# dfm/tinygp

Hardware: AMD Instinct MI355X
Metric: GP log_probability evals/sec + Cholesky TFLOP/s (fp64), N=16,384 (higher is better)
Workload: dtype f64; 1 GPU; c2: 1.5^2 ExpSquared(2.5), 1-D X, N=16384, fp64, diag=0.01, constant-density synthetic inputs (SURVEY 8d), dense Cholesky + tri-solve; n=16384, d=1, parallelism=single, nb_outer=1024

## Files before the change

### tinygp_amd/csrc/capi.hip

```cpp
#include <cmath>
#include <cstdlib>
#include <chrono>
#include <cstring>
#include <string>

#include "tgp_common.h"
#define CHAIN_HD __host__ __device__
#include "chain_tasks.h"
#define TILE_HD
#include "tile_order.h"

namespace tgp {

static thread_local std::string g_error;

void set_error(const char* fmt, ...) {
  char buf[1024];
  va_list ap;
  va_start(ap, fmt);
  vsnprintf(buf, sizeof(buf), fmt, ap);
  va_end(ap);
  g_error = buf;
}

// ... 35 lines not shown
struct tgp_solver {
  tgp_ctx* ctx = nullptr;
  int dtype = TGP_F64;
  int64_t n = 0, npad = 0;
  int d = 1;
  void* X = nullptr;
  void* diag = nullptr;
  void* A = nullptr;
  void* dinv = nullptr;
  void* vec = nullptr;
  void* vec2 = nullptr;
  void* resid = nullptr;
  void* scratch = nullptr;
  void* Minv = nullptr;
  void* winv = nullptr;
  bool winv_valid = false;
  size_t scratch_bytes = 0;
  KProg kp{};
  bool has_prog = false, factored = false, has_resid = false;
  int32_t info = 0;
  double logdet_half = 0;
  double ms[8] = {0, 0, 0, 0, 0, 0, 0, 0};
};

#define CTX_GUARD(ctx)                                                \
  TGP_ARG_CHECK((ctx) != nullptr, "null context");                    \
  std::unique_lock<std::recursive_mutex> _tgp_lock((ctx)->mu);        \
  TGP_HIP_TRY(hipSetDevice((ctx)->device))

#define SOLVER_GUARD(s)                                               \
  TGP_ARG_CHECK((s) != nullptr && (s)->ctx != nullptr, "null solver"); \
  std::unique_lock<std::recursive_mutex> _tgp_lock((s)->ctx->mu);     \
  TGP_HIP_TRY(hipSetDevice((s)->ctx->device))

template <typename T>
static int assemble_lower(tgp_ctx* ctx, const tgp::KProg& kp, int64_t n, int d, const T* X,
                          const T* diag, T* A, int64_t npad) {
  using namespace tgp;
  const int64_t tc = npad / 128;
  int64_t t1 = tc;
  if (ctx->lookahead != 0 && ctx->asm_stream != nullptr) {
    int64_t nb = ctx->nb_outer / 128;
    if (nb < 1) nb = 1;
    nb = std::max<int64_t>(nb, first_panel_cols(ctx, npad) / 128);
    if (nb < tc) t1 = nb;
  }
  const int flags = KMAT_LOWER | KMAT_PAD_IDENTITY;
  if (t1 < tc) {
    TGP_TRY(ev_record(ctx, ctx->ev_asm, ctx->stream));
    TGP_TRY(st_wait(ctx, ctx->asm_stream, ctx->ev_asm));
  }
  TGP_TRY(launch_kmat_cols<T>(ctx, ctx->stream, kp, n, n, d, X, X, diag, A, npad, npad, npad, flags, 0, t1));
  if (t1 < tc) {
    auto side = [=]() -> int {
      TGP_TRY(launch_kmat_cols<T>(ctx, ctx->asm_stream, kp, n, n, d, X, X, diag, A, npad, npad, npad,
                                  flags, t1, tc - t1));
      return ev_record(ctx, ctx->ev_asm, ctx->asm_stream);
    };
    if (ctx->asm_defer != 0) {
      ctx->deferred_asm = side;
    } else {
      TGP_TRY(side());
    }
    ctx->asm_pending = true;
  }
  return TGP_OK;
}

template <typename T>
static int ensure_winv(tgp_solver* s) {
  if (s->winv_valid) return TGP_OK;
// ... 167 lines not shown
  if (!strcmp(key, "chain_batch_minrows")) return &ctx->chain_batch_minrows;
  if (!strcmp(key, "kmat_plain_div")) return &ctx->kmat_plain_div;
  if (!strcmp(key, "chain_reserve")) return &ctx->chain_reserve;
  if (!strcmp(key, "gate_split")) return &ctx->gate_split;
  if (!strcmp(key, "reserve_max_tiles")) return &ctx->reserve_max_tiles;
  if (!strcmp(key, "sub_panel")) return &ctx->sub_panel;
  if (!strcmp(key, "sub_panel_min_rows")) return &ctx->sub_panel_min_rows;
  if (!strcmp(key, "nb_first")) return &ctx->nb_first;
  if (!strcmp(key, "split_tail")) return &ctx->split_tail;
  if (!strcmp(key, "gemm_role")) return &ctx->gemm_role;
  if (!strcmp(key, "host_join")) return &ctx->host_join;
  if (!strcmp(key, "late_join")) return &ctx->late_join;
  if (!strcmp(key, "chain_reduce")) return &ctx->chain_reduce;
  if (!strcmp(key, "asm_defer")) return &ctx->asm_defer;
  if (!strcmp(key, "tile_band")) return &ctx->tile_band;
  if (!strcmp(key, "fault_inject")) return &ctx->fault_inject;
  if (!strcmp(key, "poll_timeout_ms")) return &ctx->poll_timeout_ms;
  if (!strcmp(key, "timeout_retries")) return &ctx->timeout_retries;
  return nullptr;
}

static int set_option_checked(tgp_ctx* ctx, const char* key, int64_t value, int64_t* old) {
  int64_t* slot = option_slot(ctx, key);
  TGP_ARG_CHECK(slot != nullptr, "unknown option '%s'", key);
  if (slot == &ctx->nb_outer)
    TGP_ARG_CHECK(value >= TILE && value % TILE == 0, "nb_outer must be a positive multiple of %d", TILE);
  if (slot == &ctx->sub_panel || slot == &ctx->nb_first)
    TGP_ARG_CHECK(value >= 0 && value % TILE == 0, "%s must be a multiple of %d (0: off)", key, TILE);
  if (slot == &ctx->chain_batch) TGP_ARG_CHECK(value >= 0 && value <= 32, "chain_batch must be in [0, 32]");
  if (slot == &ctx->chain_batch_lag) TGP_ARG_CHECK(value >= 1 && value <= 64, "chain_batch_lag must be in [1, 64]");
// ... 245 lines not shown
  s->n = n;
  s->npad = round_up(n, TILE);
  s->d = d;
  const size_t es = esize(dtype);
  auto fail = [&](int code) { tgp_solver_destroy(s); return code; };
#define S_TRY(expr) do { hipError_t _e = (expr); if (_e != hipSuccess) { \
    set_error("%s failed: %s", #expr, hipGetErrorString(_e));            \
    return fail(_e == hipErrorOutOfMemory ? TGP_E_NOMEM : TGP_E_HIP); } } while (0)
  S_TRY(hipMalloc(&s->X, size_t(n) * d * es));
  S_TRY(hipMalloc(&s->diag, size_t(n) * es));
  S_TRY(hipMalloc(&s->A, size_t(s->npad) * s->npad * es));
  S_TRY(hipMalloc(&s->dinv, size_t(s->npad / TILE) * 2048 * es));
  S_TRY(hipMalloc(&s->vec, size_t(s->npad) * es));
  S_TRY(hipMalloc(&s->vec2, size_t(s->npad) * es));
  S_TRY(hipMalloc(&s->resid, size_t(s->npad) * es));
  S_TRY(hipMemcpyAsync(s->X, X_host, size_t(n) * d * es, hipMemcpyHostToDevice, ctx->stream));
  S_TRY(hipMemcpyAsync(s->diag, noise_diag_host, size_t(n) * es, hipMemcpyHostToDevice, ctx->stream));
  S_TRY(hipMemsetAsync(s->vec, 0, size_t(s->npad) * es, ctx->stream));
  S_TRY(hipMemsetAsync(s->vec2, 0, size_t(s->npad) * es, ctx->stream));
  S_TRY(hipMemsetAsync(s->resid, 0, size_t(s->npad) * es, ctx->stream));
  S_TRY(hipStreamSynchronize(ctx->stream));
#undef S_TRY
  *out = s;
  return TGP_OK;
}

int tgp_solver_destroy(tgp_solver* s) {
  if (!s) return TGP_OK;
  if (s->ctx) {
    hipSetDevice(s->ctx->device);
    hipStreamSynchronize(s->ctx->stream);
  }
  void* bufs[] = {s->X, s->diag, s->A, s->dinv, s->vec, s->vec2, s->resid, s->scratch, s->Minv, s->winv};
  for (void* b : bufs)
    if (b) hipFree(b);
  delete s;
  return TGP_OK;
}

int tgp_solver_set_noise(tgp_solver* s, const void* noise_diag_host) {
  SOLVER_GUARD(s);
  TGP_ARG_CHECK(noise_diag_host != nullptr, "null input array");
  TGP_HIP_TRY(hipMemcpyAsync(s->diag, noise_diag_host, size_t(s->n) * esize(s->dtype),
                             hipMemcpyHostToDevice, s->ctx->stream));
  TGP_HIP_TRY(hipStreamSynchronize(s->ctx->stream));
  return TGP_OK;
}

// ... 61 lines not shown
    TGP_HIP_TRY(hipEventCreate(&e2));
    TGP_HIP_TRY(hipEventRecord(e0, ctx->stream));
  }
  int status = dispatch(s->dtype, [&](auto tag) {
    using T = decltype(tag);
    T* A = (T*)s->A;
    if (fused) {
      if (resid_host) {
        TGP_TRY(upload_vec(s, s->vec, resid_host));
      } else {
        TGP_ARG_CHECK(s->has_resid, "no resident residual: call tgp_solver_set_resid first");
        TGP_HIP_TRY(hipMemcpyAsync(s->vec, s->resid, size_t(s->npad) * es, hipMemcpyDeviceToDevice,
                                   ctx->stream));
      }
    }
    if (cov_host != nullptr) {
      TGP_TRY(solver_scratch(s, size_t(s->n) * s->n * es));
      TGP_HIP_TRY(hipMemcpyAsync(s->scratch, cov_host, size_t(s->n) * s->n * es,
                                 hipMemcpyHostToDevice, ctx->stream));
      TGP_TRY(launch_set_lower_from_rowmajor<T>(ctx, s->n, s->npad, (const T*)s->scratch, A, s->npad));
    } else {
      TGP_TRY(assemble_lower<T>(ctx, s->kp, s->n, s->d, (const T*)s->X, (const T*)s->diag, A, s->npad));
    }
    if (prof) TGP_HIP_TRY(hipEventRecord(e1, ctx->stream));
    int32_t inf = 0;
    ctx->defer_join = ctx->late_join != 0;
    ctx->join_deferred = false;
    reductions_begin(ctx, s->npad, fused != 0);
    int st = potrf<T>(ctx, s->npad, A, s->npad, (T*)s->dinv, &inf, fused ? (T*)s->vec : (T*)nullptr);
    ctx->defer_join = false;
    const bool reduce = reductions_end(ctx);
    if (st < 0) return st;
    s->info = inf;
    if (prof) TGP_HIP_TRY(hipEventRecord(e2, ctx->stream));
    if (reduce) {
      TGP_TRY(launch_sum_log_diag<T>(ctx, s->n, A, s->npad, 1));
      if (fused) TGP_TRY(launch_sum_squares<T>(ctx, s->n, (const T*)s->vec, 0));
    }
    return TGP_OK;
  });
  if (status < 0) return status;
  double two[2] = {0, 0};
  int32_t inf_late = 0;
  const bool late = ctx->join_deferred;
// ... 582 lines not shown
```

### tinygp_amd/csrc/chol.hip

```cpp
#include <algorithm>
#include <atomic>
#include <functional>
#include <type_traits>

#include <thread>

#include "tgp_common.h"
#define CHAIN_HD __host__ __device__
#include "chain_tasks.h"

namespace tgp {

namespace {

typedef double d4 __attribute__((ext_vector_type(4)));
typedef float f4 __attribute__((ext_vector_type(4)));

template <typename T> struct Mfma;
template <> struct Mfma<double> {
  using acc_t = d4;
  static __device__ __forceinline__ acc_t mma(double a, double b, acc_t c) {
    return __builtin_amdgcn_mfma_f64_16x16x4f64(a, b, c, 0, 0, 0);
  }
  static __device__ __forceinline__ int drow(int lane, int r) { return (lane >> 4) + 4 * r; }
// ... 2318 lines not shown
      TGP_TRY(launch_trsv_fwd_step<T>(ctx, S2, mb, Ljj, ld, dj, y + j0));
    }
    if (need_mid) TGP_TRY(mid(ctx->ev_d));
    if (SB > 0 && j0 + TILE == sub_end && sub_end < k0 + kb) {
      const int64_t s0 = sub_end - SB, mr = n - sub_end, ncr = k0 + kb - sub_end;
      const T* P = A + s0 * ld + sub_end;
      const int64_t tiles = (mr / TILE) * (ncr / TILE) - (ncr / TILE) * (ncr / TILE - 1) / 2;
      TGP_TRY(launch_gemm_nt<T>(ctx, st, mr, ncr, SB, P, ld, P, ld, A + sub_end * ld + sub_end, ld, 1, 0,
                                tiles <= ctx->first_small_tiles ? 4 : 1));
    }
  }
  return TGP_OK;
}

template <typename T>
int potrf(tgp_ctx* ctx, int64_t n, T* A, int64_t ld, T* dinv, int32_t* info_host, T* y) {
  TGP_ARG_CHECK(n % TILE == 0 && ld >= n, "potrf: n must be a multiple of %d and ld >= n", TILE);
  if (info_host) *info_host = 0;
  if (n == 0) return TGP_OK;
  ctx->potf2_wait_counter = nullptr;
  ctx->prefix_hint_cols = 0;
  ctx->prefix_hint_counter = nullptr;
  ctx->reserve_hint = 0;
  hipStream_t S0 = ctx->stream, S1 = ctx->panel_stream;
  if (ctx->solve_on_update == 0 && y != nullptr) TGP_TRY(ensure_solve_stream(ctx));
  hipStream_t S2 = ctx->solve_on_update != 0 ? ctx->update_stream : ctx->solve_stream;
  if (y != nullptr) {
    TGP_TRY(ev_record(ctx, ctx->ev_c, S0));
    TGP_TRY(st_wait(ctx, S2, ctx->ev_c));
  }
  int64_t NB = ctx->nb_outer;
  if (NB < TILE) NB = TILE;
  NB = NB / TILE * TILE;
  if (!ctx->trace) TGP_HIP_TRY(hipMemsetAsync(ctx->d_info, 0, sizeof(int32_t), S0));
  ctx->chain_stamp_base = 0;
  ctx->chain_launches = 0;
  ctx->chain_polls_pending = false;
  const bool prof_on = ctx->profile != 0 && !ctx->trace;
// ... 9 lines not shown
  auto potf2_at = [&](hipStream_t st, int64_t j0, bool pend) -> int {
    return panel_potf2<T>(ctx, st, A, ld, dinv, 0, j0, pend);
  };
  auto panel = [&](hipStream_t st, int64_t k0, int64_t kb, bool head_done, int64_t after_blocks,
                   const std::function<int(hipEvent_t)>& mid) -> int {
    return panel_chain<T>(ctx, st, n, A, ld, dinv, 0, k0, kb, head_done, y, after_blocks, mid);
  };
  const std::function<int(hipEvent_t)> no_mid = [](hipEvent_t) { return TGP_OK; };
  auto trailing = [&](hipStream_t sq, int64_t m, int64_t nn, int64_t kb, const T* P, T* C, int role) -> int {
    ProfSpan sp{};
    const bool prof = prof_on && role != 4 && role != 5;
    if (prof) {
      TGP_TRY(prof_event(ctx, &sp.e0));
      TGP_TRY(prof_event(ctx, &sp.e1));
      TGP_HIP_TRY(hipEventRecord(sp.e0, sq));
    }
    TGP_TRY(launch_gemm_nt<T>(ctx, sq, m, nn, kb, P, ld, P, ld, C, ld, 1, 0, role));
    if (prof) {
      TGP_HIP_TRY(hipEventRecord(sp.e1, sq));
      const double entries = double(nn) * double(m) - double(nn) * double(nn - 1) / 2.0;
      sp.flops = 2.0 * entries * double(kb);
      spans.push_back(sp);
    }
    return TGP_OK;
  };

  auto join_assembly = [&]() -> int {
    TGP_TRY(run_deferred_asm(ctx, nullptr));
    if (ctx->asm_pending) {
      TGP_TRY(st_wait(ctx, S0, ctx->ev_asm));
// ... 524 lines not shown
}

#define TGP_INST(T)                                                                              \
  template int spd_inverse_lower<T>(tgp_ctx*, int64_t, const T*, int64_t, const T*, T*, int64_t); \
  template int symmetrize_lower<T>(tgp_ctx*, int64_t, T*, int64_t);                               \
  template int launch_potf2<T>(tgp_ctx*, hipStream_t, T*, int64_t, T*, int32_t*, int32_t,       \
                               const T*, int64_t);       \
  template int launch_trsm<T>(tgp_ctx*, hipStream_t, int64_t, const T*, int64_t, const T*, T*,   \
                              int64_t);                                                          \
  template int launch_panel_step<T>(tgp_ctx*, hipStream_t, int64_t, T*, int64_t, T*, int32_t*, int32_t, \
                                    const T*, bool);                                             \
  template int compute_dinv<T>(tgp_ctx*, int64_t, const T*, int64_t, T*);                        \
  template int panel_potf2<T>(tgp_ctx*, hipStream_t, T*, int64_t, T*, int64_t, int64_t, bool);   \
  template int panel_chain<T>(tgp_ctx*, hipStream_t, int64_t, T*, int64_t, T*, int64_t, int64_t, \
                              int64_t, bool, T*, int64_t, const std::function<int(hipEvent_t)>&, int64_t, int64_t); \
  template int potrf<T>(tgp_ctx*, int64_t, T*, int64_t, T*, int32_t*, T*);                           \
  template int trsv<T>(tgp_ctx*, int64_t, const T*, int64_t, const T*, int, T*, const T*, const T*); \
  template int compute_winv<T>(tgp_ctx*, int64_t, const T*, int64_t, T*);                        \
  template int gemv_sub<T>(tgp_ctx*, int64_t, int64_t, const T*, int64_t, const T*, T*);                          \
  template int trsm_right_lt<T>(tgp_ctx*, int64_t, int64_t, const T*, int64_t, const T*, T*,     \
                                int64_t);
TGP_INST(float)
TGP_INST(double)
#undef TGP_INST

}
```

### tinygp_amd/csrc/gemm.hip

```cpp
#include <type_traits>

#include "tgp_common.h"

#define TILE_HD __host__ __device__
#include "tile_order.h"

namespace tgp {

namespace {

typedef double d4 __attribute__((ext_vector_type(4)));
typedef float f4 __attribute__((ext_vector_type(4)));

template <typename T> struct Mfma;
template <> struct Mfma<double> {
  using acc_t = d4;
  using v2_t = double __attribute__((ext_vector_type(2)));
  static __device__ __forceinline__ acc_t mma(double a, double b, acc_t c) {
    return __builtin_amdgcn_mfma_f64_16x16x4f64(a, b, c, 0, 0, 0);
  }
  static __device__ __forceinline__ int drow(int lane, int r) { return (lane >> 4) + 4 * r; }
};
template <> struct Mfma<float> {
  using acc_t = f4;
// ... 15 lines not shown
  int tm, tn;
  int k;
  int lower;
  int mode;
  int nblk;
  int skip00;
  int dG, dr, dl0, dnbt;
  int split_first, split_s, ngrid;
  T* ws;
  int* cnt;
  int batch;
  int64_t sA, sB, sC;
  int band;
  int prefix_tn = 0, prefix_cnt = 0;
  int32_t* prefix_done = nullptr;
};

__device__ __forceinline__ void decode_tile(int b, int tm, int tn, int lower, int& ti, int& tj, int band = 0) {
  tile_decode(b, tm, tn, lower, band, ti, tj);
}

template <typename T>
__device__ __forceinline__ void decode_tile_dist(int b, const GemmArgs<T>& g, int& ti, int& tj, int& gt) {
  int q = 0, g0 = (g.dl0 * g.dG + g.dr) * g.dnbt;
  const int step = g.dG * g.dnbt, tri = g.dnbt * (g.dnbt - 1) / 2;
  for (;;) {
    const int cnt = g.dnbt * (g.tm - g0) - tri;
    if (b < cnt) break;
    b -= cnt;
    g0 += step;
    ++q;
// ... 72 lines not shown
      ti += g.prefix_tn;
      tj += g.prefix_tn;
    }
    gt = tj;
  } else {
    decode_tile(bid, g.tm, g.tn, g.lower, ti, tj, g.band);
    gt = tj;
  }

  const int tid = threadIdx.x, lane = tid & 63, w = tid >> 6;
  const int wr = w >> 1, wc = w & 1;
  const int64_t i0 = int64_t(ti) * BM, j0 = int64_t(tj) * BN;

  int nkt = (g.mode & 2) ? ((g.k < (tj + 1) * BN ? g.k : (tj + 1) * BN) / BK) : g.k / BK;
  if (ROLE == 3 && (g.mode & 8)) nkt = (g.k < (ti + 1) * BM ? g.k : (ti + 1) * BM) / BK;
  const int kt0 = (g.mode & 4) ? (ti * BM) / BK : 0;
  const bool krev = ROLE == 3 && (g.mode & 16);
  const int lrow = lane & 15, lk = lane >> 4;
  T* Cb = gC + (j0 + wc * 64) * g.ldc + i0 + wr * 64;

  if constexpr (sizeof(T) == 8) {
    const int lq = (lane >> 2) & 3, lj = lane & 3;
    double acc[4][4][4];
#pragma unroll
    for (int a = 0; a < 4; ++a)
#pragma unroll
      for (int b = 0; b < 4; ++b)
#pragma unroll
        for (int t = 0; t < 4; ++t) acc[a][b][t] = 0.0;
    int rot[4];
#pragma unroll
    for (int t = 0; t < 4; ++t) rot[t] = 4 * ((lq + t) & 3) + lj;

    constexpr int NCH = 8;
    const int kq = (nkt - kt0) / nsl;
    const int kbeg = kt0 + slice * kq, kend = kbeg + kq;
    const bool pipe = (g.mode == 0) && nsl == 1 && (kend - kbeg >= NCH);
    double cst[8];
    const int wu = __builtin_amdgcn_readfirstlane(w);
    const char* Cu = reinterpret_cast<const char*>(gC + (j0 + (wu & 1) * 64) * g.ldc + i0 + (wu >> 1) * 64);
    uint32_t voff[4];
#pragma unroll
    for (int t = 0; t < 4; ++t) voff[t] = uint32_t((int64_t(4 * lq + lk) * g.ldc + rot[t]) * 8);
    const uint32_t lds_a = uint32_t(size_t((__attribute__((address_space(3))) T*)(&sA[0][0]))) + uint32_t(wu * LDS_LD * 8);
    const uint32_t lds_b = uint32_t(size_t((__attribute__((address_space(3))) T*)(&sB[0][0]))) + uint32_t(wu * LDS_LD * 8);
    const T* Au = gA + i0;
    const T* Bu = gB + int64_t(gt) * BN;
    const uint32_t lane16 = uint32_t(lane) * 16u;
    auto issue_tile = [&](int kt_, int buf_) {
      const int64_t kg = int64_t(krev ? kbeg + kend - 1 - kt_ : kt_) * BK + wu;
#pragma unroll
// ... 38 lines not shown
#pragma unroll
            for (int t = 0; t < 4; ++t)
              acc[a][b][t] = __builtin_amdgcn_mfma_f64_4x4x4f64(aop[a], bop[t], acc[a][b][t], 0, 0, NEG);
        }
      }
      tile_landed();
      __syncthreads();
      if constexpr (c >= 0) {
        __builtin_amdgcn_sched_barrier(0);
#pragma unroll
        for (int bb = 0; bb < 2; ++bb)
#pragma unroll
          for (int t = 0; t < 4; ++t) acc[c >> 1][(c & 1) * 2 + bb][t] += cst[bb * 4 + t];
      }
    };
    issue_tile(kbeg, kbeg & 1);
    tile_landed();
    __syncthreads();
    int kt = kbeg;
    if (pipe) {
      int one = 1;
      asm volatile("" : "+s"(one));
#define TGP_STAGED(C) \
  for (int q = 0; q < one; ++q, ++kt) ktile(kt, std::integral_constant<int, C>{}, std::true_type{});
      TGP_STAGED(0) TGP_STAGED(1) TGP_STAGED(2) TGP_STAGED(3) TGP_STAGED(4)
      TGP_STAGED(5) TGP_STAGED(6) TGP_STAGED(7)
#undef TGP_STAGED
      for (; kt < kend; ++kt) ktile(kt, std::integral_constant<int, -1>{}, std::true_type{});
    } else {
      for (; kt < kend; ++kt) ktile(kt, std::integral_constant<int, -1>{}, std::false_type{});
    }
// ... 481 lines not shown
static unsigned persistent_grid(const tgp_ctx* ctx, int nblk, int64_t reserve) {
  if (reserve <= 0) return unsigned(nblk);
  int64_t slots = 2 * int64_t(ctx->cus > 0 ? ctx->cus : 256) - reserve;
  slots = slots / 8 * 8;
  if (slots < 8) slots = 8;
  return unsigned(nblk <= slots ? nblk : slots);
}

template <typename T>
int launch_gemm_nt(tgp_ctx* ctx, hipStream_t st, int64_t m, int64_t n, int64_t k, const T* A,
                   int64_t lda, const T* B, int64_t ldb, T* C, int64_t ldc, int lower, int mode,
                   int role) {
  TGP_ARG_CHECK(m % BM == 0 && n % BN == 0 && k % BK == 0 && k > 0,
                "gemm_nt: m,n must be multiples of %d and k of %d (got %lld,%lld,%lld)", BM, BK,
                (long long)m, (long long)n, (long long)k);
  if (m == 0 || n == 0) return TGP_OK;
  if (ctx->trace) {
    const int64_t pfx = role == 0 ? ctx->prefix_hint_cols / BN : 0;
    ctx->prefix_hint_cols = 0;
    ctx->prefix_hint_counter = nullptr;
    if (role == 0) ctx->reserve_hint = 0;
    trace_push(ctx, 3, st, trace_off(ctx, A), trace_off(ctx, B), trace_off(ctx, C), m, n, k,
               int64_t(lower) | (int64_t(role) << 8) | (pfx << 16), ldc);
    return TGP_OK;
  }
  GemmArgs<T> g;
  g.skip00 = 0;
  g.dG = g.dr = g.dl0 = g.dnbt = 0;
  g.split_first = 0; g.split_s = 1; g.ngrid = 0; g.ws = nullptr; g.cnt = nullptr;
  g.batch = 1; g.sA = g.sB = g.sC = 0;
// ... 27 lines not shown
  } else {
    g.nblk = g.tm * g.tn;
  }
  const int64_t reserve = role == 0 ? ctx->reserve_hint : 0;
  ctx->reserve_hint = 0;
  if (role == 0 && ctx->prefix_hint_cols > 0) {
    TGP_ARG_CHECK(lower && mode == 0 && m == n && ctx->prefix_hint_cols % BN == 0 && ctx->prefix_hint_cols < n &&
                      k / BK >= 8 && ctx->prefix_hint_counter != nullptr,
                  "gemm_nt: a prefix needs a lower square update with at least 128 k-columns");
    g.prefix_tn = int(ctx->prefix_hint_cols / BN);
    g.prefix_cnt = tile_count(g.tm, g.prefix_tn, 1);
    g.prefix_done = ctx->prefix_hint_counter;
  }
  ctx->prefix_hint_cols = 0;
  ctx->prefix_hint_counter = nullptr;
  g.split_first = g.nblk; g.split_s = 1; g.ngrid = g.nblk; g.ws = nullptr; g.cnt = nullptr;
  if (ctx->split_tail != 0 && role == 0 && mode == 0 && reserve <= 0 && sizeof(T) == 8 && st == ctx->stream && g.prefix_cnt == 0) {
    const int slots = 2 * (ctx->cus > 0 ? ctx->cus : 256);
    const int R = g.nblk % slots, nkt = g.k / BK;
    int S = 1;
    while (R > 0 && 2 * S * R <= slots && 2 * S <= 8 && nkt % (2 * S) == 0 && nkt / (2 * S) >= 8) S *= 2;
    if (S > 1) {
      const size_t need = size_t(slots) * BM * BN * sizeof(T) + size_t(slots) * sizeof(int);
      if (ctx->gemm_ws_bytes < need) {
        if (ctx->d_gemm_ws) TGP_HIP_TRY(hipFree(ctx->d_gemm_ws));
        ctx->d_gemm_ws = nullptr;
        ctx->gemm_ws_bytes = 0;
        TGP_HIP_TRY(hipMalloc(&ctx->d_gemm_ws, need));
        TGP_HIP_TRY(hipMemset(ctx->d_gemm_ws, 0, need));
        ctx->gemm_ws_bytes = need;
// ... 136 lines not shown
```

### tinygp_amd/csrc/kmat.hip

```cpp
#include <algorithm>

#include "tgp_common.h"

namespace tgp {

namespace {

template <typename T> struct MathC;
template <> struct MathC<double> {
  static constexpr double SQRT3 = 1.7320508075688772;
  static constexpr double SQRT5 = 2.23606797749979;
  static constexpr double PI = 3.141592653589793;
  static constexpr double TWO_PI = 6.283185307179586;
};
template <> struct MathC<float> {
  static constexpr float SQRT3 = 1.7320508075688772f;
  static constexpr float SQRT5 = 2.23606797749979f;
  static constexpr float PI = 3.141592653589793f;
  static constexpr float TWO_PI = 6.283185307179586f;
};

template <typename T, int FAM = 0>
__device__ __forceinline__ T leaf_value(const KProg& kp, int i, T r1, T r2, T r3 = T(0)) {
  const int op = kp.op[i];
// ... 278 lines not shown
      const T a = MathC<T>::SQRT3 * by_p0.template div<FAST>(dist);
      return (T(1) + a) * exp(-a);
    } else {
      const T a = MathC<T>::SQRT5 * by_p0.template div<FAST>(dist);
      return (T(1) + a + by3.template div<FAST>(a * a)) * exp(-a);
    }
  }
}

template <typename T, int OP, int L2>
__device__ __forceinline__ T leaf_fast(T r1, T r2, T p0, T p0sq) {
  const UDiv<T> by_p0(p0), by_p0sq(p0sq), by3(T(3));
  return leaf_fast<T, OP, L2, false>(r1, r2, by_p0, by_p0sq, by3);
}

template <typename T, int D, int OP, int L2>
__global__ __launch_bounds__(256) void kmat_fast_kernel(T p0, T amp, int64_t n1, int64_t n2,
                                                        const T* __restrict__ X1,
                                                        const T* __restrict__ X2,
                                                        const T* __restrict__ diag, T* __restrict__ out,
                                                        int64_t ld, int flags, int tc0, int tri_h) {
  typedef T T2 __attribute__((ext_vector_type(2)));
  constexpr int NCOL = 32;
  const int cq = threadIdx.x >> 6, l = threadIdx.x & 63;
  int tr, tc;
  if (flags & KMAT_LOWER) {
    const int b = blockIdx.x;
    const double h2 = 2.0 * tri_h + 1.0;
    int j = int((h2 - sqrt(h2 * h2 - 8.0 * double(b))) * 0.5);
    while (j > 0 && j * tri_h - j * (j - 1) / 2 > b) --j;
    while ((j + 1) * tri_h - (j + 1) * j / 2 <= b) ++j;
    tc = tc0 + j;
    tr = tc + (b - (j * tri_h - j * (j - 1) / 2));
  } else {
    tr = blockIdx.x;
    tc = blockIdx.y + tc0;
// ... 2 lines not shown
  for (int t = threadIdx.x; t < KT * D; t += 256) s2all[t] = X2[int64_t(tc) * KT * D + t];
  __syncthreads();
  const T* s2 = s2all + cq * NCOL * D;
  const int64_t c0 = int64_t(tc) * KT + cq * NCOL;
  const int64_t gi = int64_t(tr) * KT + 2 * l;
  T xr[2][D];
#pragma unroll
  for (int h = 0; h < 2; ++h)
#pragma unroll
    for (int t = 0; t < D; ++t) xr[h][t] = X1[(gi + h) * D + t];
  const bool on_diag = diag != nullptr && tr == tc;
  const T dg0 = on_diag ? diag[gi] : T(0), dg1 = on_diag ? diag[gi + 1] : T(0);
  const UDiv<T> by_p0(p0), by_p0sq(p0 * p0), by3(T(3));
  const int ldiag = 2 * l - cq * NCOL;
  T* o = out + c0 * ld + gi;
  auto columns = [&](auto fast) -> T {
    constexpr bool FAST = decltype(fast)::value;
    T seen = 0;
#pragma unroll 4
    for (int c = 0; c < NCOL; ++c) {
      T v[2];
#pragma unroll
      for (int h = 0; h < 2; ++h) {
        T r1 = 0, r2 = 0;
#pragma unroll
        for (int t = 0; t < D; ++t) {
          const T dx = xr[h][t] - s2[c * D + t];
          r1 += fabs(dx);
          r2 += dx * dx;
        }
        v[h] = amp * leaf_fast<T, OP, L2, FAST>(r1, r2, by_p0, by_p0sq, by3);
        if constexpr (FAST) seen = fmax(seen, L2 ? r2 : r1);
      }
      if (on_diag) {
        if (c == ldiag) v[0] += dg0;
        if (c == ldiag + 1) v[1] += dg1;
      }
      T2 pair;
      pair.x = v[0];
      pair.y = v[1];
      *reinterpret_cast<T2*>(o + int64_t(c) * ld) = pair;
    }
    return seen;
  };
  bool plain = true;
  if (sizeof(T) == 8 && !(flags & KMAT_PLAIN_DIV) && by_p0.exact && by_p0sq.exact) {
    plain = !(columns(std::true_type{}) <= T(0x1p300));
  }
  if (plain) columns(std::false_type{});
}

template <typename T, int D, int FAM>
__global__ __launch_bounds__(256) void kmat_kernel(KProg kp, int64_t n1, int64_t n2, int d,
                                                   const T* __restrict__ X1,
                                                   const T* __restrict__ X2,
                                                   const T* __restrict__ diag, T* __restrict__ out,
                                                   int64_t ld, int64_t rows_out, int64_t cols_out,
                                                   int flags, int tc0, int ftr, int ftc) {
  const int tr = blockIdx.x, tc = blockIdx.y + tc0;
  if ((flags & KMAT_LOWER) && tr < tc) return;
  if (tr < ftr && tc < ftc) return;
  extern __shared__ __attribute__((aligned(16))) char smem[];
  T* s1 = reinterpret_cast<T*>(smem);
  T* s2 = s1 + KT * d;
  const int64_t r0 = int64_t(tr) * KT, c0 = int64_t(tc) * KT;
  load_tile_pair(s1, s2, X1, X2, r0, c0, n1, n2, d);

  const int il = threadIdx.x & (KT - 1);
  const int g = threadIdx.x >> 7;
  const int64_t gi = r0 + il;
  T xr[D > 0 ? D : 1];
  if constexpr (D > 0) {
#pragma unroll
    for (int t = 0; t < D; ++t) xr[t] = s1[il * D + t];
  }
  const T dg = (diag != nullptr && gi < n1) ? diag[gi] : T(0);
  if (gi >= rows_out) return;
  for (int c = 0; c < KT / 2; ++c) {
    const int jl = g * (KT / 2) + c;
    const int64_t gj = c0 + jl;
    if (gj >= cols_out) break;
    T v;
    if (gi < n1 && gj < n2) {
      T r1, r2, r3;
      if constexpr (D > 0) pair_dist<T, FAM, D>(xr, s2 + jl * D, d, r1, r2, r3);
      else pair_dist<T, FAM, 0>(s1 + il * d, s2 + jl * d, d, r1, r2, r3);
      v = eval_kprog<T, FAM>(kp, r1, r2, r3);
      if (diag != nullptr && gi == gj) v += dg;
    } else {
      v = ((flags & KMAT_PAD_IDENTITY) && gi == gj) ? T(1) : T(0);
    }
    out[gj * ld + gi] = v;
  }
}

template <typename T, int OP, int L2>
__device__ __forceinline__ T leaf_deriv_fast(T r1, T r2, T p0) {
  if constexpr (OP == TGP_K_EXPSQ) {
    const T sq = L2 ? r2 : r1 * r1;
    return exp(T(-0.5) * (sq / (p0 * p0))) * sq / (p0 * p0 * p0);
  } else {
    const T dist = L2 ? ((r2 == T(0)) ? r1 : sqrt(r2)) : r1;
    if constexpr (OP == TGP_K_EXP) {
      return exp(-dist / p0) * dist / (p0 * p0);
    } else if constexpr (OP == TGP_K_M32) {
      const T a = MathC<T>::SQRT3 * (dist / p0);
      return a * a * exp(-a) / p0;
// ... 281 lines not shown

template <int MAXD, typename F>
static void with_dim(int d, F&& f) {
  if (d == 1) f(IC<1>{});
  else if (d == 2) f(IC<2>{});
  else if (d == 3) f(IC<3>{});
  else if constexpr (MAXD == 4) {
    if (d == 4) f(IC<4>{});
    else f(IC<0>{});
  }
}

template <typename T>
int launch_kmat_cols(tgp_ctx* ctx, hipStream_t st, const KProg& kp, int64_t n1, int64_t n2, int d,
                     const T* X1, const T* X2, const T* diag, T* out, int64_t ld, int64_t rows_out,
                     int64_t cols_out, int flags, int64_t tc0, int64_t ntc) {
  TGP_ARG_CHECK(d >= 1 && d <= TGP_MAX_DIM, "input dimension must be 1..%d (got %d)", TGP_MAX_DIM, d);
  TGP_ARG_CHECK(rows_out >= n1 && cols_out >= n2 && ld >= rows_out, "kmat: bad output extents");
  if (rows_out == 0 || cols_out == 0 || ntc <= 0) return TGP_OK;
  const int64_t tr = (rows_out + KT - 1) / KT, tc = (cols_out + KT - 1) / KT;
  TGP_ARG_CHECK(tc0 >= 0 && tc0 + ntc <= tc, "kmat: column tile range outside the matrix");
  if (ctx->trace) {
    trace_push(ctx, 7, st, tc0, ntc, ld, flags);
    return TGP_OK;
  }
  TGP_ARG_CHECK(ntc <= 65535, "kmat: too many column tiles");
  int ftr = 0, ftc = 0;
  const FastProg fp = fast_prog(kp);
  if (fp.op >= 0 && d <= 3 && ld % 2 == 0 && reinterpret_cast<uintptr_t>(out) % 16 == 0) {
    ftr = int(n1 / KT);
    ftc = int(n2 / KT);
    const int64_t fc = std::min<int64_t>(tc0 + ntc, ftc) - tc0;
    const int64_t tri_h = (flags & KMAT_LOWER) ? ftr - tc0 : 0;
    const int64_t tri_c = std::min<int64_t>(fc, tri_h);
    const bool any = (flags & KMAT_LOWER) ? (tri_c > 0) : (ftr > 0 && fc > 0);
    if (any) {
      dim3 fgrid((unsigned)ftr, (unsigned)fc);
      if (flags & KMAT_LOWER) fgrid = dim3((unsigned)(tri_c * tri_h - tri_c * (tri_c - 1) / 2));
      const int fflags = flags | (ctx->kmat_plain_div != 0 ? KMAT_PLAIN_DIV : 0);
      with_dim<3>(d, [&](auto dd) {
        with_fast_leaf(fp, [&](auto op, auto l2) {
          constexpr int D = decltype(dd)::value, OP = decltype(op)::value, L2 = decltype(l2)::value;
          hipLaunchKernelGGL((kmat_fast_kernel<T, D, OP, L2>), fgrid, dim3(256), 0, st, T(fp.p0), T(fp.amp), n1, n2, X1,
                             X2, diag, out, ld, fflags, (int)tc0, (int)tri_h);
        });
      });
    } else {
      ftr = ftc = 0;
    }
    if (ftr == tr && ftc >= tc0 + ntc) {
      TGP_HIP_TRY(hipGetLastError());
      return TGP_OK;
    }
  }
  dim3 grid((unsigned)tr, (unsigned)ntc);
  const size_t shmem = 2 * size_t(KT) * d * sizeof(T);
  with_dim<4>(d, [&](auto dd) {
    with_family<true>(kp, [&](auto fam) {
      constexpr int D = decltype(dd)::value, FAM = decltype(fam)::value;
      hipLaunchKernelGGL((kmat_kernel<T, D, FAM>), grid, dim3(256), shmem, st, kp, n1, n2, d, X1, X2, diag, out, ld,
                         rows_out, cols_out, flags, (int)tc0, ftr, ftc);
    });
  });
  TGP_HIP_TRY(hipGetLastError());
  return TGP_OK;
}

template <typename T>
int launch_kmat(tgp_ctx* ctx, const KProg& kp, int64_t n1, int64_t n2, int d, const T* X1,
                const T* X2, const T* diag, T* out, int64_t ld, int64_t rows_out, int64_t cols_out,
                int flags) {
  return launch_kmat_cols<T>(ctx, ctx->stream, kp, n1, n2, d, X1, X2, diag, out, ld, rows_out,
                             cols_out, flags, 0, (cols_out + KT - 1) / KT);
}

template <typename T>
int launch_kdiag(tgp_ctx* ctx, const KProg& kp, int64_t n, int d, const T* X, const T* add, T* out) {
  if (n == 0) return TGP_OK;
  const dim3 grid((unsigned)((n + 255) / 256));
  if (kfamily(kp) == 2)
    TGP_ARG_CHECK(X != nullptr && d >= 1 && d <= TGP_MAX_DIM, "kdiag: a DOT program needs the points");
  with_family<false>(kp, [&](auto fam) {
    constexpr int FAM = decltype(fam)::value;
    hipLaunchKernelGGL((kdiag_kernel<T, FAM>), grid, dim3(256), 0, ctx->stream, kp, n, d, X, add, out);
  });
  TGP_HIP_TRY(hipGetLastError());
  return TGP_OK;
}
// ... 120 lines not shown
}

#define TGP_INST(T)                                                                               \
  template int launch_kgrad_cols<T>(tgp_ctx*, const KProg&, int, int, int64_t, int, const T*, const T*, const T*,   \
                                    int64_t, int64_t, int64_t, int, int, double*);                                  \
  template int launch_kcols_diag<T>(tgp_ctx*, int64_t, const T*, int64_t, int64_t, T*);                            \
  template int launch_kgrad<T>(tgp_ctx*, const KProg&, int, int, int64_t, int, const T*, const T*, \
                               const T*, int64_t, double*);                                       \
  template int launch_noise_grad<T>(tgp_ctx*, int64_t, const T*, const T*, int64_t, T*);          \
  template int launch_kgrad_fast<T>(tgp_ctx*, const KProg&, int64_t, int, const T*, const T*,     \
                                    const T*, int64_t, double*, int*, int*);                      \
  template int launch_kmat<T>(tgp_ctx*, const KProg&, int64_t, int64_t, int, const T*, const T*,  \
                              const T*, T*, int64_t, int64_t, int64_t, int);                      \
  template int launch_kmat_cols<T>(tgp_ctx*, hipStream_t, const KProg&, int64_t, int64_t, int,    \
                                   const T*, const T*, const T*, T*, int64_t, int64_t, int64_t,   \
                                   int, int64_t, int64_t);                                        \
  template int launch_kdiag<T>(tgp_ctx*, const KProg&, int64_t, int, const T*, const T*, T*);     \
  template int launch_kmat_gemv<T>(tgp_ctx*, const KProg&, int64_t, int64_t, int, const T*,       \
                                   const T*, const T*, T*);                                       \
  template int launch_kmat_gemv_multi<T>(tgp_ctx*, const KProg&, int64_t, int64_t, int, const T*, \
                                         const T*, const T*, int64_t, T*);
TGP_INST(float)
TGP_INST(double)
#undef TGP_INST

}
```

### tinygp_amd/csrc/tgp_common.h

```cpp
#pragma once

#include <hip/hip_runtime.h>

#include <cstdarg>
#include <cstdint>
#include <cstdio>
#include <chrono>
#include <array>
#include <functional>
#include <map>
#include <mutex>
#include <vector>

#include "../../include/tgp_hip.h"

namespace tgp {

constexpr int TILE = TGP_TILE;
constexpr int SUB = 16;

void set_error(const char* fmt, ...);

#define TGP_HIP_TRY(expr)                                                                  \
  do {                                                                                     \
// ... 77 lines not shown
  int64_t sub_panel_min_rows = 0;
  int64_t nb_first = 0;
  int64_t split_tail = 0;
  int64_t gemm_role = 1;
  int64_t late_join = 1;
  int64_t chain_reduce = 1;
  double* d_chain_red = nullptr;
  int64_t chain_red_total = 0;
  int64_t chain_red_written = 0;
  bool reductions_done = false;
  bool defer_join = false;
  bool join_deferred = false;
  int64_t reserve_hint = 0;
  int64_t prefix_hint_cols = 0;
  int32_t* prefix_hint_counter = nullptr;
  const int32_t* potf2_wait_counter = nullptr;
  int64_t potf2_wait_target = 0;
  uint32_t* d_step_flag = nullptr;
  uint32_t step_epoch = 0;
  int64_t chain_kernel = 1;
  uint32_t* d_chain_flags = nullptr;
  int32_t* d_chain_ticket = nullptr;
  int64_t chain_fast_update = 0;
  int64_t chain_batch = 1;
  int64_t chain_batch_lag = 1;
  int64_t chain_batch_rowlag = 4;
  int64_t chain_batch_minrows = 32;
  struct ChainTable {
    uint64_t* dev = nullptr;
    int64_t count = 0;
// ... 118 lines not shown
  ctx->reductions_done = false;
  return launch;
}

int ensure_dinv(tgp_ctx* ctx, size_t bytes);
int ensure_work(tgp_ctx* ctx, size_t bytes);
int ensure_solve_stream(tgp_ctx* ctx);

template <typename T>
int launch_kmat(tgp_ctx* ctx, const KProg& kp, int64_t n1, int64_t n2, int d, const T* X1,
                const T* X2, const T* diag, T* out, int64_t ld, int64_t rows_out, int64_t cols_out,
                int flags);
template <typename T>
int launch_kmat_cols(tgp_ctx* ctx, hipStream_t st, const KProg& kp, int64_t n1, int64_t n2, int d,
                     const T* X1, const T* X2, const T* diag, T* out, int64_t ld, int64_t rows_out,
                     int64_t cols_out, int flags, int64_t tc0, int64_t ntc);
constexpr int KMAT_LOWER = 1;
constexpr int KMAT_PAD_IDENTITY = 2;
constexpr int KMAT_PLAIN_DIV = 4;

template <typename T>
int launch_kdiag(tgp_ctx* ctx, const KProg& kp, int64_t n, int d, const T* X, const T* add, T* out);
template <typename T>
int launch_kmat_gemv(tgp_ctx* ctx, const KProg& kp, int64_t n1, int64_t n2, int d, const T* X1,
                     const T* X2, const T* v, T* out);
template <typename T>
int launch_kmat_gemv_multi(tgp_ctx* ctx, const KProg& kp, int64_t n1, int64_t n2, int d, const T* X1,
                           const T* X2, const T* v, int64_t nv, T* out);

template <typename T>
int launch_gemm_nt(tgp_ctx* ctx, hipStream_t st, int64_t m, int64_t n, int64_t k, const T* A,
// ... 32 lines not shown
int64_t poll_limit_ms();
int join_bounded(tgp_ctx* ctx, hipStream_t st, int64_t n);
int run_deferred_asm(tgp_ctx* ctx, hipStream_t behind);
template <typename T>
int panel_potf2(tgp_ctx* ctx, hipStream_t st, T* A, int64_t ld, T* dinv, int64_t pivot_off,
                int64_t j0, bool pend);
template <typename T>
int panel_chain(tgp_ctx* ctx, hipStream_t st, int64_t n, T* A, int64_t ld, T* dinv,
                int64_t pivot_off, int64_t k0, int64_t kb, bool head_done, T* y,
                int64_t after_blocks, const std::function<int(hipEvent_t)>& mid, int64_t blk_begin = 0,
                int64_t blk_end = -1);
template <typename T>
int launch_trsv_fwd_step(tgp_ctx* ctx, hipStream_t st, int64_t m_below, const T* Ljj, int64_t ld,
                         const T* dj, T* yj);
template <typename T>
int potrf(tgp_ctx* ctx, int64_t n, T* A, int64_t ld, T* dinv, int32_t* info_host, T* y = nullptr);
template <typename T>
int trsv(tgp_ctx* ctx, int64_t n, const T* L, int64_t ld, const T* dinv, int transpose, T* y,
         const T* winv = nullptr, const T* yin = nullptr);
template <typename T>
int compute_winv(tgp_ctx* ctx, int64_t n, const T* L, int64_t ld, T* winv);
template <typename T>
int trsm_right_lt(tgp_ctx* ctx, int64_t m, int64_t n, const T* L, int64_t ldl, const T* dinv,
                  T* B, int64_t ldb);
template <typename T>
int gemv_sub(tgp_ctx* ctx, int64_t m, int64_t k, const T* P, int64_t ld, const T* x, T* y);
template <typename T>
int spd_inverse_lower(tgp_ctx* ctx, int64_t n, const T* L, int64_t ldl, const T* winv, T* S, int64_t lds);
template <typename T>
int symmetrize_lower(tgp_ctx* ctx, int64_t n, T* A, int64_t ld);
template <typename T>
// ... 43 lines not shown
```

Before: 39.46 evals/s.

## Track exact-zero tile envelope during assembly and skip zero k-ranges in trailing GEMM

The kernel-matrix assembly kernels now record, per 128x128 tile, whether any entry is nonzero into a byte table. In the Cholesky trailing update GEMM, each output tile looks up the first nonzero column tile of its two row blocks and starts the k-loop there, skipping work on exactly-zero blocks, or skips the tile entirely. With an ExpSquared kernel of small lengthscale, far-off-diagonal entries underflow to exact zero in fp64, so the factor keeps a band envelope and much of the trailing-update work can be dropped. This costs an extra reduction in assembly and envelope lookups in the GEMM. The feature is on by default, relies on exact zeros in the assembled matrix, and adds complexity to the split-k paths.

```diff
diff --git a/tinygp_amd/csrc/capi.hip b/tinygp_amd/csrc/capi.hip
--- a/tinygp_amd/csrc/capi.hip
+++ b/tinygp_amd/csrc/capi.hip
@@ -73,6 +73,7 @@
   void* scratch = nullptr;
   void* Minv = nullptr;
   void* winv = nullptr;
+  uint8_t* env = nullptr;
   bool winv_valid = false;
   size_t scratch_bytes = 0;
   KProg kp{};
@@ -94,7 +95,7 @@
 
 template <typename T>
 static int assemble_lower(tgp_ctx* ctx, const tgp::KProg& kp, int64_t n, int d, const T* X,
-                          const T* diag, T* A, int64_t npad) {
+                          const T* diag, T* A, int64_t npad, uint8_t* env = nullptr) {
   using namespace tgp;
   const int64_t tc = npad / 128;
   int64_t t1 = tc;
@@ -109,11 +110,11 @@
     TGP_TRY(ev_record(ctx, ctx->ev_asm, ctx->stream));
     TGP_TRY(st_wait(ctx, ctx->asm_stream, ctx->ev_asm));
   }
-  TGP_TRY(launch_kmat_cols<T>(ctx, ctx->stream, kp, n, n, d, X, X, diag, A, npad, npad, npad, flags, 0, t1));
+  TGP_TRY(launch_kmat_cols<T>(ctx, ctx->stream, kp, n, n, d, X, X, diag, A, npad, npad, npad, flags, 0, t1, env, tc));
   if (t1 < tc) {
     auto side = [=]() -> int {
       TGP_TRY(launch_kmat_cols<T>(ctx, ctx->asm_stream, kp, n, n, d, X, X, diag, A, npad, npad, npad,
-                                  flags, t1, tc - t1));
+                                  flags, t1, tc - t1, env, tc));
       return ev_record(ctx, ctx->ev_asm, ctx->asm_stream);
     };
     if (ctx->asm_defer != 0) {
@@ -311,6 +312,7 @@
   if (!strcmp(key, "chain_reduce")) return &ctx->chain_reduce;
   if (!strcmp(key, "asm_defer")) return &ctx->asm_defer;
   if (!strcmp(key, "tile_band")) return &ctx->tile_band;
+  if (!strcmp(key, "envelope")) return &ctx->envelope;
   if (!strcmp(key, "fault_inject")) return &ctx->fault_inject;
   if (!strcmp(key, "poll_timeout_ms")) return &ctx->poll_timeout_ms;
   if (!strcmp(key, "timeout_retries")) return &ctx->timeout_retries;
@@ -586,6 +588,7 @@
   S_TRY(hipMalloc(&s->vec, size_t(s->npad) * es));
   S_TRY(hipMalloc(&s->vec2, size_t(s->npad) * es));
   S_TRY(hipMalloc(&s->resid, size_t(s->npad) * es));
+  S_TRY(hipMalloc(&s->env, size_t(s->npad / TILE) * size_t(s->npad / TILE)));
   S_TRY(hipMemcpyAsync(s->X, X_host, size_t(n) * d * es, hipMemcpyHostToDevice, ctx->stream));
   S_TRY(hipMemcpyAsync(s->diag, noise_diag_host, size_t(n) * es, hipMemcpyHostToDevice, ctx->stream));
   S_TRY(hipMemsetAsync(s->vec, 0, size_t(s->npad) * es, ctx->stream));
@@ -603,7 +606,7 @@
     hipSetDevice(s->ctx->device);
     hipStreamSynchronize(s->ctx->stream);
   }
-  void* bufs[] = {s->X, s->diag, s->A, s->dinv, s->vec, s->vec2, s->resid, s->scratch, s->Minv, s->winv};
+  void* bufs[] = {s->X, s->diag, s->A, s->dinv, s->vec, s->vec2, s->resid, s->scratch, s->Minv, s->winv, s->env};
   for (void* b : bufs)
     if (b) hipFree(b);
   delete s;
@@ -695,20 +698,22 @@
                                    ctx->stream));
       }
     }
+    uint8_t* env = nullptr;
     if (cov_host != nullptr) {
       TGP_TRY(solver_scratch(s, size_t(s->n) * s->n * es));
       TGP_HIP_TRY(hipMemcpyAsync(s->scratch, cov_host, size_t(s->n) * s->n * es,
                                  hipMemcpyHostToDevice, ctx->stream));
       TGP_TRY(launch_set_lower_from_rowmajor<T>(ctx, s->n, s->npad, (const T*)s->scratch, A, s->npad));
     } else {
-      TGP_TRY(assemble_lower<T>(ctx, s->kp, s->n, s->d, (const T*)s->X, (const T*)s->diag, A, s->npad));
+      if (ctx->envelope != 0) env = s->env;
+      TGP_TRY(assemble_lower<T>(ctx, s->kp, s->n, s->d, (const T*)s->X, (const T*)s->diag, A, s->npad, env));
     }
     if (prof) TGP_HIP_TRY(hipEventRecord(e1, ctx->stream));
     int32_t inf = 0;
     ctx->defer_join = ctx->late_join != 0;
     ctx->join_deferred = false;
     reductions_begin(ctx, s->npad, fused != 0);
-    int st = potrf<T>(ctx, s->npad, A, s->npad, (T*)s->dinv, &inf, fused ? (T*)s->vec : (T*)nullptr);
+    int st = potrf<T>(ctx, s->npad, A, s->npad, (T*)s->dinv, &inf, fused ? (T*)s->vec : (T*)nullptr, env);
     ctx->defer_join = false;
     const bool reduce = reductions_end(ctx);
     if (st < 0) return st;
diff --git a/tinygp_amd/csrc/chol.hip b/tinygp_amd/csrc/chol.hip
--- a/tinygp_amd/csrc/chol.hip
+++ b/tinygp_amd/csrc/chol.hip
@@ -2356,7 +2356,7 @@
 }
 
 template <typename T>
-int potrf(tgp_ctx* ctx, int64_t n, T* A, int64_t ld, T* dinv, int32_t* info_host, T* y) {
+int potrf(tgp_ctx* ctx, int64_t n, T* A, int64_t ld, T* dinv, int32_t* info_host, T* y, const uint8_t* env) {
   TGP_ARG_CHECK(n % TILE == 0 && ld >= n, "potrf: n must be a multiple of %d and ld >= n", TILE);
   if (info_host) *info_host = 0;
   if (n == 0) return TGP_OK;
@@ -2364,6 +2364,7 @@
   ctx->prefix_hint_cols = 0;
   ctx->prefix_hint_counter = nullptr;
   ctx->reserve_hint = 0;
+  ctx->env_hint = nullptr;
   hipStream_t S0 = ctx->stream, S1 = ctx->panel_stream;
   if (ctx->solve_on_update == 0 && y != nullptr) TGP_TRY(ensure_solve_stream(ctx));
   hipStream_t S2 = ctx->solve_on_update != 0 ? ctx->update_stream : ctx->solve_stream;
@@ -2403,6 +2404,13 @@
       TGP_TRY(prof_event(ctx, &sp.e0));
       TGP_TRY(prof_event(ctx, &sp.e1));
       TGP_HIP_TRY(hipEventRecord(sp.e0, sq));
+    }
+    if (env != nullptr && role == 0 && kb % TILE == 0) {
+      const int64_t coff = C - A, poff = P - A;
+      ctx->env_hint = env;
+      ctx->env_hint_ld = n / TILE;
+      ctx->env_hint_row0 = (coff % ld) / TILE;
+      ctx->env_hint_col0 = (poff / ld) / TILE;
     }
     TGP_TRY(launch_gemm_nt<T>(ctx, sq, m, nn, kb, P, ld, P, ld, C, ld, 1, 0, role));
     if (prof) {
@@ -2957,7 +2965,7 @@
   template int panel_potf2<T>(tgp_ctx*, hipStream_t, T*, int64_t, T*, int64_t, int64_t, bool);   \
   template int panel_chain<T>(tgp_ctx*, hipStream_t, int64_t, T*, int64_t, T*, int64_t, int64_t, \
                               int64_t, bool, T*, int64_t, const std::function<int(hipEvent_t)>&, int64_t, int64_t); \
-  template int potrf<T>(tgp_ctx*, int64_t, T*, int64_t, T*, int32_t*, T*);                           \
+  template int potrf<T>(tgp_ctx*, int64_t, T*, int64_t, T*, int32_t*, T*, const uint8_t*);                           \
   template int trsv<T>(tgp_ctx*, int64_t, const T*, int64_t, const T*, int, T*, const T*, const T*); \
   template int compute_winv<T>(tgp_ctx*, int64_t, const T*, int64_t, T*);                        \
   template int gemv_sub<T>(tgp_ctx*, int64_t, int64_t, const T*, int64_t, const T*, T*);                          \
diff --git a/tinygp_amd/csrc/gemm.hip b/tinygp_amd/csrc/gemm.hip
--- a/tinygp_amd/csrc/gemm.hip
+++ b/tinygp_amd/csrc/gemm.hip
@@ -53,7 +53,19 @@
   int band;
   int prefix_tn = 0, prefix_cnt = 0;
   int32_t* prefix_done = nullptr;
+  const uint8_t* env = nullptr;
+  int env_ld = 0, env_r0 = 0, env_c0 = 0;
 };
+
+__device__ __forceinline__ int env_first(const uint8_t* env, int env_ld, int R, int lim, int lane) {
+  const uint8_t* row = env + int64_t(R) * env_ld;
+  for (int c0 = 0; c0 < lim; c0 += 64) {
+    const int c = c0 + lane;
+    const unsigned long long m = __ballot(c < lim && row[c] != 0);
+    if (m != 0) return c0 + __builtin_ctzll(m);
+  }
+  return lim;
+}
 
 __device__ __forceinline__ void decode_tile(int b, int tm, int tn, int lower, int& ti, int& tj, int band = 0) {
   tile_decode(b, tm, tn, lower, band, ti, tj);
@@ -156,11 +168,32 @@
 
   int nkt = (g.mode & 2) ? ((g.k < (tj + 1) * BN ? g.k : (tj + 1) * BN) / BK) : g.k / BK;
   if (ROLE == 3 && (g.mode & 8)) nkt = (g.k < (ti + 1) * BM ? g.k : (ti + 1) * BM) / BK;
-  const int kt0 = (g.mode & 4) ? (ti * BM) / BK : 0;
+  int kt0 = (g.mode & 4) ? (ti * BM) / BK : 0;
+  bool env_cut = false;
+  if constexpr (ROLE == 0 || ROLE == 2) {
+    if (g.env != nullptr) {
+      const int lim = g.env_c0 + g.k / BM;
+      const int fi = env_first(g.env, g.env_ld, g.env_r0 + ti, lim, threadIdx.x & 63);
+      const int fj = ti == tj ? fi : env_first(g.env, g.env_ld, g.env_r0 + tj, lim, threadIdx.x & 63);
+      const int f = fi > fj ? fi : fj;
+      if (f > g.env_c0) {
+        kt0 = (f - g.env_c0 - ((nsl == 1 && f < lim && sizeof(T) == 8) ? 1 : 0)) * (BM / BK);
+        env_cut = true;
+      }
+    }
+  }
   const bool krev = ROLE == 3 && (g.mode & 16);
   const int lrow = lane & 15, lk = lane >> 4;
   T* Cb = gC + (j0 + wc * 64) * g.ldc + i0 + wr * 64;
 
+  if constexpr (ROLE == 0 || ROLE == 2) {
+    if (env_cut && kt0 >= nkt && !(ROLE == 2 && nsl > 1)) {
+      if (ROLE == 0 && in_prefix && threadIdx.x == 0)
+        __hip_atomic_fetch_add(g.prefix_done, 1, __ATOMIC_RELAXED, __HIP_MEMORY_SCOPE_AGENT);
+      continue;
+    }
+  }
+
   if constexpr (sizeof(T) == 8) {
     const int lq = (lane >> 2) & 3, lj = lane & 3;
     double acc[4][4][4];
@@ -175,8 +208,11 @@
     for (int t = 0; t < 4; ++t) rot[t] = 4 * ((lq + t) & 3) + lj;
 
     constexpr int NCH = 8;
-    const int kq = (nkt - kt0) / nsl;
-    const int kbeg = kt0 + slice * kq, kend = kbeg + kq;
+    const int kt00 = (nsl > 1 && env_cut) ? 0 : kt0;
+    const int kq = (nkt - kt00) / nsl;
+    const int kend = kt00 + (slice + 1) * kq;
+    int kbeg = kt00 + slice * kq;
+    if (nsl > 1 && env_cut && kbeg < kt0) kbeg = kt0 < kend ? kt0 : kend;
     const bool pipe = (g.mode == 0) && nsl == 1 && (kend - kbeg >= NCH);
     double cst[8];
     const int wu = __builtin_amdgcn_readfirstlane(w);
@@ -245,7 +281,7 @@
           for (int t = 0; t < 4; ++t) acc[c >> 1][(c & 1) * 2 + bb][t] += cst[bb * 4 + t];
       }
     };
-    issue_tile(kbeg, kbeg & 1);
+    issue_tile(kbeg < kend ? kbeg : kend - 1, kbeg & 1);
     tile_landed();
     __syncthreads();
     int kt = kbeg;
@@ -757,6 +793,8 @@
   TGP_ARG_CHECK(m % BM == 0 && n % BN == 0 && k % BK == 0 && k > 0,
                 "gemm_nt: m,n must be multiples of %d and k of %d (got %lld,%lld,%lld)", BM, BK,
                 (long long)m, (long long)n, (long long)k);
+  const uint8_t* env = ctx->env_hint;
+  ctx->env_hint = nullptr;
   if (m == 0 || n == 0) return TGP_OK;
   if (ctx->trace) {
     const int64_t pfx = role == 0 ? ctx->prefix_hint_cols / BN : 0;
@@ -814,6 +852,13 @@
   }
   ctx->prefix_hint_cols = 0;
   ctx->prefix_hint_counter = nullptr;
+  if (env != nullptr && role == 0 && lower && mode == 0 && A == B && lda == ldb && k % BM == 0) {
+    g.env = env;
+    g.env_ld = int(ctx->env_hint_ld);
+    g.env_r0 = int(ctx->env_hint_row0);
+    g.env_c0 = int(ctx->env_hint_col0);
+    TGP_ARG_CHECK(g.env_r0 + g.tm <= g.env_ld && g.env_c0 + g.k / BM <= g.env_r0, "gemm_nt: envelope outside its table");
+  }
   g.split_first = g.nblk; g.split_s = 1; g.ngrid = g.nblk; g.ws = nullptr; g.cnt = nullptr;
   if (ctx->split_tail != 0 && role == 0 && mode == 0 && reserve <= 0 && sizeof(T) == 8 && st == ctx->stream && g.prefix_cnt == 0) {
     const int slots = 2 * (ctx->cus > 0 ? ctx->cus : 256);
diff --git a/tinygp_amd/csrc/kmat.hip b/tinygp_amd/csrc/kmat.hip
--- a/tinygp_amd/csrc/kmat.hip
+++ b/tinygp_amd/csrc/kmat.hip
@@ -316,12 +316,16 @@
   return leaf_fast<T, OP, L2, false>(r1, r2, by_p0, by_p0sq, by3);
 }
 
+__device__ __forceinline__ bool any_bit(double v) { return __double_as_longlong(v) != 0; }
+__device__ __forceinline__ bool any_bit(float v) { return __float_as_uint(v) != 0u; }
+
 template <typename T, int D, int OP, int L2>
 __global__ __launch_bounds__(256) void kmat_fast_kernel(T p0, T amp, int64_t n1, int64_t n2,
                                                         const T* __restrict__ X1,
                                                         const T* __restrict__ X2,
                                                         const T* __restrict__ diag, T* __restrict__ out,
-                                                        int64_t ld, int flags, int tc0, int tri_h) {
+                                                        int64_t ld, int flags, int tc0, int tri_h,
+                                                        uint8_t* __restrict__ env, int64_t env_ld) {
   typedef T T2 __attribute__((ext_vector_type(2)));
   constexpr int NCOL = 32;
   const int cq = threadIdx.x >> 6, l = threadIdx.x & 63;
@@ -354,8 +358,10 @@
   const UDiv<T> by_p0(p0), by_p0sq(p0 * p0), by3(T(3));
   const int ldiag = 2 * l - cq * NCOL;
   T* o = out + c0 * ld + gi;
+  bool nz = false;
   auto columns = [&](auto fast) -> T {
     constexpr bool FAST = decltype(fast)::value;
+    nz = false;
     T seen = 0;
 #pragma unroll 4
     for (int c = 0; c < NCOL; ++c) {
@@ -379,6 +385,7 @@
       T2 pair;
       pair.x = v[0];
       pair.y = v[1];
+      nz = nz || any_bit(v[0]) || any_bit(v[1]);
       *reinterpret_cast<T2*>(o + int64_t(c) * ld) = pair;
     }
     return seen;
@@ -388,6 +395,10 @@
     plain = !(columns(std::true_type{}) <= T(0x1p300));
   }
   if (plain) columns(std::false_type{});
+  if (env != nullptr) {
+    const int any = __syncthreads_or(nz ? 1 : 0);
+    if (threadIdx.x == 0) env[int64_t(tr) * env_ld + tc] = any ? 1 : 0;
+  }
 }
 
 template <typename T, int D, int FAM>
@@ -396,7 +407,8 @@
                                                    const T* __restrict__ X2,
                                                    const T* __restrict__ diag, T* __restrict__ out,
                                                    int64_t ld, int64_t rows_out, int64_t cols_out,
-                                                   int flags, int tc0, int ftr, int ftc) {
+                                                   int flags, int tc0, int ftr, int ftc,
+                                                   uint8_t* __restrict__ env, int64_t env_ld) {
   const int tr = blockIdx.x, tc = blockIdx.y + tc0;
   if ((flags & KMAT_LOWER) && tr < tc) return;
   if (tr < ftr && tc < ftc) return;
@@ -415,11 +427,11 @@
     for (int t = 0; t < D; ++t) xr[t] = s1[il * D + t];
   }
   const T dg = (diag != nullptr && gi < n1) ? diag[gi] : T(0);
-  if (gi >= rows_out) return;
+  bool nz = false;
   for (int c = 0; c < KT / 2; ++c) {
     const int jl = g * (KT / 2) + c;
     const int64_t gj = c0 + jl;
-    if (gj >= cols_out) break;
+    if (gi >= rows_out || gj >= cols_out) break;
     T v;
     if (gi < n1 && gj < n2) {
       T r1, r2, r3;
@@ -431,6 +443,11 @@
       v = ((flags & KMAT_PAD_IDENTITY) && gi == gj) ? T(1) : T(0);
     }
     out[gj * ld + gi] = v;
+    nz = nz || any_bit(v);
+  }
+  if (env != nullptr) {
+    const int any = __syncthreads_or(nz ? 1 : 0);
+    if (threadIdx.x == 0) env[int64_t(tr) * env_ld + tc] = any ? 1 : 0;
   }
 }
 
@@ -742,12 +759,13 @@
 template <typename T>
 int launch_kmat_cols(tgp_ctx* ctx, hipStream_t st, const KProg& kp, int64_t n1, int64_t n2, int d,
                      const T* X1, const T* X2, const T* diag, T* out, int64_t ld, int64_t rows_out,
-                     int64_t cols_out, int flags, int64_t tc0, int64_t ntc) {
+                     int64_t cols_out, int flags, int64_t tc0, int64_t ntc, uint8_t* env, int64_t env_ld) {
   TGP_ARG_CHECK(d >= 1 && d <= TGP_MAX_DIM, "input dimension must be 1..%d (got %d)", TGP_MAX_DIM, d);
   TGP_ARG_CHECK(rows_out >= n1 && cols_out >= n2 && ld >= rows_out, "kmat: bad output extents");
   if (rows_out == 0 || cols_out == 0 || ntc <= 0) return TGP_OK;
   const int64_t tr = (rows_out + KT - 1) / KT, tc = (cols_out + KT - 1) / KT;
   TGP_ARG_CHECK(tc0 >= 0 && tc0 + ntc <= tc, "kmat: column tile range outside the matrix");
+  TGP_ARG_CHECK(env == nullptr || env_ld >= tc, "kmat: envelope table narrower than the matrix");
   if (ctx->trace) {
     trace_push(ctx, 7, st, tc0, ntc, ld, flags);
     return TGP_OK;
@@ -770,7 +788,7 @@
         with_fast_leaf(fp, [&](auto op, auto l2) {
           constexpr int D = decltype(dd)::value, OP = decltype(op)::value, L2 = decltype(l2)::value;
           hipLaunchKernelGGL((kmat_fast_kernel<T, D, OP, L2>), fgrid, dim3(256), 0, st, T(fp.p0), T(fp.amp), n1, n2, X1,
-                             X2, diag, out, ld, fflags, (int)tc0, (int)tri_h);
+                             X2, diag, out, ld, fflags, (int)tc0, (int)tri_h, env, env_ld);
         });
       });
     } else {
@@ -787,7 +805,7 @@
     with_family<true>(kp, [&](auto fam) {
       constexpr int D = decltype(dd)::value, FAM = decltype(fam)::value;
       hipLaunchKernelGGL((kmat_kernel<T, D, FAM>), grid, dim3(256), shmem, st, kp, n1, n2, d, X1, X2, diag, out, ld,
-                         rows_out, cols_out, flags, (int)tc0, ftr, ftc);
+                         rows_out, cols_out, flags, (int)tc0, ftr, ftc, env, env_ld);
     });
   });
   TGP_HIP_TRY(hipGetLastError());
@@ -799,7 +817,7 @@
                 const T* X2, const T* diag, T* out, int64_t ld, int64_t rows_out, int64_t cols_out,
                 int flags) {
   return launch_kmat_cols<T>(ctx, ctx->stream, kp, n1, n2, d, X1, X2, diag, out, ld, rows_out,
-                             cols_out, flags, 0, (cols_out + KT - 1) / KT);
+                             cols_out, flags, 0, (cols_out + KT - 1) / KT, nullptr, 0);
 }
 
 template <typename T>
@@ -950,7 +968,7 @@
                               const T*, T*, int64_t, int64_t, int64_t, int);                      \
   template int launch_kmat_cols<T>(tgp_ctx*, hipStream_t, const KProg&, int64_t, int64_t, int,    \
                                    const T*, const T*, const T*, T*, int64_t, int64_t, int64_t,   \
-                                   int, int64_t, int64_t);                                        \
+                                   int, int64_t, int64_t, uint8_t*, int64_t);                     \
   template int launch_kdiag<T>(tgp_ctx*, const KProg&, int64_t, int, const T*, const T*, T*);     \
   template int launch_kmat_gemv<T>(tgp_ctx*, const KProg&, int64_t, int64_t, int, const T*,       \
                                    const T*, const T*, T*);                                       \
diff --git a/tinygp_amd/csrc/tgp_common.h b/tinygp_amd/csrc/tgp_common.h
--- a/tinygp_amd/csrc/tgp_common.h
+++ b/tinygp_amd/csrc/tgp_common.h
@@ -115,6 +115,9 @@
   int64_t reserve_hint = 0;
   int64_t prefix_hint_cols = 0;
   int32_t* prefix_hint_counter = nullptr;
+  int64_t envelope = 1;
+  const uint8_t* env_hint = nullptr;
+  int64_t env_hint_ld = 0, env_hint_row0 = 0, env_hint_col0 = 0;
   const int32_t* potf2_wait_counter = nullptr;
   int64_t potf2_wait_target = 0;
   uint32_t* d_step_flag = nullptr;
@@ -263,7 +266,8 @@
 template <typename T>
 int launch_kmat_cols(tgp_ctx* ctx, hipStream_t st, const KProg& kp, int64_t n1, int64_t n2, int d,
                      const T* X1, const T* X2, const T* diag, T* out, int64_t ld, int64_t rows_out,
-                     int64_t cols_out, int flags, int64_t tc0, int64_t ntc);
+                     int64_t cols_out, int flags, int64_t tc0, int64_t ntc, uint8_t* env = nullptr,
+                     int64_t env_ld = 0);
 constexpr int KMAT_LOWER = 1;
 constexpr int KMAT_PAD_IDENTITY = 2;
 constexpr int KMAT_PLAIN_DIV = 4;
@@ -326,7 +330,8 @@
 int launch_trsv_fwd_step(tgp_ctx* ctx, hipStream_t st, int64_t m_below, const T* Ljj, int64_t ld,
                          const T* dj, T* yj);
 template <typename T>
-int potrf(tgp_ctx* ctx, int64_t n, T* A, int64_t ld, T* dinv, int32_t* info_host, T* y = nullptr);
+int potrf(tgp_ctx* ctx, int64_t n, T* A, int64_t ld, T* dinv, int32_t* info_host, T* y = nullptr,
+          const uint8_t* env = nullptr);
 template <typename T>
 int trsv(tgp_ctx* ctx, int64_t n, const T* L, int64_t ld, const T* dinv, int transpose, T* y,
          const T* winv = nullptr, const T* yin = nullptr);
```

Result: no change. 39.54 evals/s, median of 6 (+0.2%).
